# tk1363704/CAREL-VAE

Measured on AMD Instinct MI355X. Metric: clause-pairs/sec (training step), higher is better.
Workload: dtype bf16

## Files before the change

carel_vae_amd/csrc/rowvec_device.h:

```cpp
#pragma once
#include "carel_hip_internal.h"

namespace carel {

constexpr int TH = 768;
constexpr int TNV = TH / 256;

struct PtrSet4 { const float* w[4]; const float* b[4]; };

template <int ACT>
__global__ __launch_bounds__(256) void rowvec_linear_kernel(const float* __restrict__ in, long in_stride, const int* __restrict__ row_idx,
                                                            int B, int N, int seg, PtrSet4 ps, float* __restrict__ out, long out_stride) {
  const int lane = threadIdx.x & 63;
  const int n = blockIdx.x * 4 + (threadIdx.x >> 6);
  if (n >= N) return;
  const int bg = (B + gridDim.y - 1) / gridDim.y, b0 = blockIdx.y * bg, b1 = min(B, b0 + bg);
  const float* w = ps.w[n / seg] + (long)(n % seg) * TH;
  const float bias = ps.b[n / seg] ? ps.b[n / seg][n % seg] : 0.f;
  float4 wv[TNV];
#pragma unroll
  for (int i = 0; i < TNV; ++i) wv[i] = *(const float4*)(w + (i * 64 + lane) * 4);
  for (int b = b0; b < b1; b += 4) {
    float s[4];
#pragma unroll
    for (int u = 0; u < 4; ++u) {
      const int bb = min(b + u, b1 - 1);
      const float* x = row_idx ? in + (long)row_idx[bb] * TH : in + (long)bb * in_stride;
      float t = 0.f;
#pragma unroll
      for (int i = 0; i < TNV; ++i) {
        const float4 xv = *(const float4*)(x + (i * 64 + lane) * 4);
        t += (xv.x * wv[i].x + xv.y * wv[i].y) + (xv.z * wv[i].z + xv.w * wv[i].w);
      }
      s[u] = t;
    }
#pragma unroll
    for (int off = 32; off > 0; off >>= 1) {
#pragma unroll
      for (int u = 0; u < 4; ++u) s[u] += __shfl_xor(s[u], off, 64);
    }
#pragma unroll
    for (int u = 0; u < 4; ++u) {
      float v = s[u] + bias;
      if (ACT == 1) v = tanhf(v);
      if (lane == 0 && b + u < b1) out[(long)(b + u) * out_stride + n] = v;
    }
  }
}

struct OutSet4 { float* w[4]; float* b[4]; };
static __global__ __launch_bounds__(256) void rowvec_wgrad_kernel(const float* __restrict__ dY, long dy_stride, const float* __restrict__ X,
                                                           long x_stride, const int* __restrict__ row_idx, int B, int N, int seg, OutSet4 os) {
  const int lane = threadIdx.x & 63;
  const int n = blockIdx.x * 4 + (threadIdx.x >> 6);
  if (n >= N) return;
  float4 acc[TNV];
#pragma unroll
  for (int i = 0; i < TNV; ++i) acc[i] = float4{0.f, 0.f, 0.f, 0.f};
  float sb = 0.f;
  constexpr int U = 8;
  for (int b = 0; b < B; b += U) {
    float g[U]; float4 xv[U][TNV];
#pragma unroll
    for (int u = 0; u < U; ++u) {
      const int bb = min(b + u, B - 1);
      g[u] = (b + u < B) ? dY[(long)bb * dy_stride + n] : 0.f;
      const float* x = row_idx ? X + (long)row_idx[bb] * TH : X + (long)bb * x_stride;
#pragma unroll
      for (int i = 0; i < TNV; ++i) xv[u][i] = *(const float4*)(x + (i * 64 + lane) * 4);
    }
#pragma unroll
    for (int u = 0; u < U; ++u) {
      sb += g[u];
#pragma unroll
      for (int i = 0; i < TNV; ++i) {
        acc[i].x = fmaf(g[u], xv[u][i].x, acc[i].x); acc[i].y = fmaf(g[u], xv[u][i].y, acc[i].y);
        acc[i].z = fmaf(g[u], xv[u][i].z, acc[i].z); acc[i].w = fmaf(g[u], xv[u][i].w, acc[i].w);
      }
    }
  }
  float* w = os.w[n / seg] + (long)(n % seg) * TH;
#pragma unroll
  for (int i = 0; i < TNV; ++i) *(float4*)(w + (i * 64 + lane) * 4) = acc[i];
  if (lane == 0 && os.b[n / seg]) os.b[n / seg][n % seg] = sb;
}

constexpr int DG_CHUNK = 32;
template <int MODE>
__global__ __launch_bounds__(256) void rowvec_dgrad_kernel(const float* __restrict__ dY, long dy_stride, int B, int N, int seg,
                                                           PtrSet4 ps, const float* __restrict__ y, float* __restrict__ dpre,
                                                           float* __restrict__ part) {
  const int lane = threadIdx.x & 63;
  const int b = blockIdx.x * 4 + (threadIdx.x >> 6);
  if (b >= B) return;
  float4 acc[TNV];
#pragma unroll
  for (int i = 0; i < TNV; ++i) acc[i] = float4{0.f, 0.f, 0.f, 0.f};
  const int n0 = blockIdx.y * DG_CHUNK, n1 = min(N, n0 + DG_CHUNK);
  constexpr int U = 8;
  for (int nb = n0; nb < n1; nb += U) {
    float g[U]; float4 wv[U][TNV];
#pragma unroll
    for (int u = 0; u < U; ++u) {
      const int n = min(nb + u, n1 - 1);
      float gg = (nb + u < n1) ? dY[(long)b * dy_stride + n] : 0.f;
      if (MODE == 1) {
        const float yy = y[(long)b * N + n];
        gg *= (1.0f - yy * yy);
        if (lane == 0 && nb + u < n1) dpre[(long)b * N + n] = gg;
      }
      g[u] = gg;
      const float* w = ps.w[n / seg] + (long)(n % seg) * TH;
#pragma unroll
      for (int i = 0; i < TNV; ++i) wv[u][i] = *(const float4*)(w + (i * 64 + lane) * 4);
    }
#pragma unroll
    for (int u = 0; u < U; ++u) {
#pragma unroll
      for (int i = 0; i < TNV; ++i) {
        acc[i].x = fmaf(g[u], wv[u][i].x, acc[i].x); acc[i].y = fmaf(g[u], wv[u][i].y, acc[i].y);
        acc[i].z = fmaf(g[u], wv[u][i].z, acc[i].z); acc[i].w = fmaf(g[u], wv[u][i].w, acc[i].w);
      }
    }
  }
  float* o = part + ((long)blockIdx.y * B + b) * TH;
#pragma unroll
  for (int i = 0; i < TNV; ++i) *(float4*)(o + (i * 64 + lane) * 4) = acc[i];
}

static __global__ __launch_bounds__(256) void sum_parts_kernel(const float* __restrict__ part, float* __restrict__ out, long n, int nparts) {
  const long i = ((long)blockIdx.x * 256 + threadIdx.x) * 4;
  if (i >= n) return;
  float4 a = *(const float4*)(part + i);
  for (int p = 1; p < nparts; ++p) {
    const float4 b = *(const float4*)(part + (long)p * n + i);
    a.x += b.x; a.y += b.y; a.z += b.z; a.w += b.w;
  }
  *(float4*)(out + i) = a;
}

static __global__ void scale_inplace_kernel(float* __restrict__ x, long n, const float* __restrict__ scale) {
  const float s = scale[0];
  long i = (long)blockIdx.x * blockDim.x + threadIdx.x;
  const long stride = (long)gridDim.x * blockDim.x;
  for (; i < n; i += stride) x[i] *= s;
}
static __global__ __launch_bounds__(256) void scatter_cls_kernel(const float* __restrict__ dcls, int B, int S, const int* __restrict__ row_idx,
                                                          float* __restrict__ dx) {
  const int b = blockIdx.x;
  const long row = row_idx ? (long)row_idx[b] : (long)b * S;
  for (int k = threadIdx.x; k < TH; k += 256) dx[row * TH + k] = dcls[(long)b * TH + k];
}


}
```

carel_vae_amd/csrc/tail.hip:

```cpp
#include "carel_hip_internal.h"
#include "mmd_device.h"
#include "hsic_device.h"
#include "rowvec_device.h"

namespace carel {

struct TailCore {
  int B, D, EC;
  const float* lat;
  const float* eps_e; const float* eps_c;
  const float* emo_w; const float* emo_b;
  const float* cau_w; const float* cau_b;
  const float* pair_w; const float* pair_b;
  const long* emo_labels; const float* cau_labels; const float* pair_labels;
  float w_mmd, w_emo, w_cau, w_pair, kl_w, ls;
  int dis_mode;
  int emo_bce;
  Dropout d_emo, d_cau, d_pair;
  float alpha, mmd_eps;
  const float* label_sum_override; float n_override;
  int label_sum_ranks;
  const float* z_global; int n_global, row_offset; float mmd_grad_scale;
  int rank_stride;
  const float* mmd_part; int mmd_nblk; const float* dz_mmd;
// ... 350 lines not shown
  float ls;
  float* part;
  float* rowstat;
  float* dz_part;
  float* dw; float* db;
  float gscale;
};

template <int CD2>
__device__ __forceinline__ float dec_logit(const float* wr, const float* zrow, int D2rt, float bias) {
  const int D2 = CD2 ? CD2 : D2rt;
  float s = bias;
  if (CD2 && (CD2 & 3) == 0) {
#pragma unroll
    for (int k = 0; k < D2; k += 4) {
      const float4 zv = *(const float4*)(zrow + k);
      s = fmaf(wr[k], zv.x, s); s = fmaf(wr[k + 1], zv.y, s); s = fmaf(wr[k + 2], zv.z, s); s = fmaf(wr[k + 3], zv.w, s);
    }
  } else {
#pragma unroll
    for (int k = 0; k < D2; ++k) s = fmaf(wr[k], zrow[k], s);
  }
  return s;
}

template <int PASS, int CD2>
__global__ __launch_bounds__(DEC_J * DEC_MAXG) void decoder_kernel(DecArgs a) {
  const int D2 = CD2 ? CD2 : a.D2;
  const int ws = D2 + 1;
  extern __shared__ __attribute__((aligned(16))) char smem_raw[];
  float* zl = (float*)smem_raw;
  float* red = zl + a.B * D2;
  float* wl = red + 16;
  float* tile = wl + DEC_J * ws;
  float* tile2 = tile + a.B * DEC_J;
  const int t = threadIdx.x, nthr = blockDim.x, G = nthr / DEC_J;
  const int tj = t & (DEC_J - 1), g = t / DEC_J;
  const int j0 = blockIdx.x * DEC_J, j = j0 + tj;
  const bool live = j < a.V;
  const int Bg = (a.B + G - 1) / G, b0 = g * Bg, b1 = min(a.B, b0 + Bg);
  for (int e = t; e < a.B * D2; e += nthr) zl[e] = a.z[e];
  {
    const int nrow = min(DEC_J, a.V - j0);
    for (int e = t; e < nrow * D2; e += nthr) { const int r = e / D2, k = e - r * D2; wl[r * ws + k] = a.w[(long)j0 * D2 + e]; }
  }
  __syncthreads();
  float wr[CD2 ? CD2 : DEC_MAXD2];
  _Pragma("unroll") for (int k = 0; k < D2; ++k) wr[k] = live ? wl[tj * ws + k] : 0.f;
  const float bias = live ? a.b[j] : 0.f;
  const int lane = t & 63, wv = t >> 6, nwv = nthr >> 6;
  if (PASS == 1) {
    for (int b = b0; b < b1; ++b) tile[b * DEC_J + tj] = live ? dec_logit<CD2>(wr, zl + b * D2, D2, bias) : -INFINITY;
    __syncthreads();
    for (int b = wv; b < a.B; b += nwv) {
      const float x0 = tile[b * DEC_J + lane], x1 = tile[b * DEC_J + 64 + lane];
      const float m = wave_max(fmaxf(x0, x1));
      const float s2 = wave_sum(expf(x0 - m) + expf(x1 - m));
      if (lane == 0) { a.part[((long)blockIdx.x * a.B + b) * 2] = m; a.part[((long)blockIdx.x * a.B + b) * 2 + 1] = s2; }
    }
  } else if (PASS == 2) {
    for (int bb = b0; bb < b1; bb += 4) {
      float bw[4];
      _Pragma("unroll") for (int u = 0; u < 4; ++u) bw[u] = (live && bb + u < b1) ? a.bow[(long)(bb + u) * a.V + j] : 0.f;
      _Pragma("unroll") for (int u = 0; u < 4; ++u) {
        const int b = bb + u;
        if (b < b1) {
          float le = 0.f, dt = 0.f;
          if (live) {
            const float lp = dec_logit<CD2>(wr, zl + b * D2, D2, bias) - a.rowstat[b * 4] - a.rowstat[b * 4 + 1];
            const float p = expf(lp);
            const float tg = bw[u] * (1.f - a.ls) + a.ls / a.V;
            le = -(tg * fmaxf(lp, -100.f) + (1.f - tg) * fmaxf(log1pf(-p), -100.f));
            dt = p * ((p - tg) / fmaxf((1.f - p) * p, 1e-12f));
          }
          tile[b * DEC_J + tj] = le; tile2[b * DEC_J + tj] = dt;
        }
      }
    }
    __syncthreads();
    for (int b = wv; b < a.B; b += nwv) {
      const float le = wave_sum(tile[b * DEC_J + lane] + tile[b * DEC_J + 64 + lane]);
      const float dt = wave_sum(tile2[b * DEC_J + lane] + tile2[b * DEC_J + 64 + lane]);
      if (lane == 0) { a.part[((long)blockIdx.x * a.B + b) * 2] = le; a.part[((long)blockIdx.x * a.B + b) * 2 + 1] = dt; }
    }
  } else {
    float dwr[CD2 ? CD2 : DEC_MAXD2];
    _Pragma("unroll") for (int k = 0; k < D2; ++k) dwr[k] = 0.f;
    float dbj = 0.f;
    for (int bb = b0; bb < b1; bb += 4) {
      float bw[4];
      _Pragma("unroll") for (int u = 0; u < 4; ++u) bw[u] = (live && bb + u < b1) ? a.bow[(long)(bb + u) * a.V + j] : 0.f;
      _Pragma("unroll") for (int u = 0; u < 4; ++u) {
        const int b = bb + u;
        if (b < b1) {
          float gg = 0.f;
          if (live) {
            const float lp = dec_logit<CD2>(wr, zl + b * D2, D2, bias) - a.rowstat[b * 4] - a.rowstat[b * 4 + 1];
            const float p = expf(lp);
            const float tg = bw[u] * (1.f - a.ls) + a.ls / a.V;
            const float gp = (p - tg) / fmaxf((1.f - p) * p, 1e-12f);
            gg = p * (gp - a.rowstat[b * 4 + 2]) * a.gscale;
            _Pragma("unroll") for (int k = 0; k < D2; ++k) dwr[k] = fmaf(gg, zl[b * D2 + k], dwr[k]);
            dbj += gg;
          }
          tile[b * DEC_J + tj] = gg;
        }
      }
    }
    float* dwp = tile2;
    float* dbp = dwp + (G - 1) * DEC_J * ws;
    if (g > 0) {
      _Pragma("unroll") for (int k = 0; k < D2; ++k) dwp[((g - 1) * DEC_J + tj) * ws + k] = dwr[k];
      dbp[(g - 1) * DEC_J + tj] = dbj;
    }
    __syncthreads();
    if (g == 0 && live) {
      for (int q = 0; q < G - 1; ++q) {
        _Pragma("unroll") for (int k = 0; k < D2; ++k) dwr[k] += dwp[(q * DEC_J + tj) * ws + k];
        dbj += dbp[q * DEC_J + tj];
      }
      _Pragma("unroll") for (int k = 0; k < D2; ++k) a.dw[(long)j * D2 + k] = dwr[k];
      a.db[j] = dbj;
    }
    for (int e = t; e < a.B * D2; e += nthr) {
      const int b = e / D2, k = e - b * D2;
      const int nrow = min(DEC_J, a.V - j0);
      float s = 0.f;
      for (int jj = 0; jj < nrow; ++jj) s = fmaf(tile[b * DEC_J + jj], wl[jj * ws + k], s);
      a.dz_part[(long)blockIdx.x * a.B * D2 + e] = s;
    }
  }
}

__global__ __launch_bounds__(256) void decoder_combine_kernel(const float* __restrict__ part, int chunks, int B, int pass,
                                                              float* __restrict__ rowstat) {
  const int lane = threadIdx.x & 63;
  const int b = blockIdx.x * 4 + (threadIdx.x >> 6);
  if (b >= B) return;
  if (pass == 1) {
    float m = -INFINITY;
    for (int c = lane; c < chunks; c += 64) m = fmaxf(m, part[((long)c * B + b) * 2]);
    m = wave_max(m);
    float s = 0.f;
    for (int c = lane; c < chunks; c += 64) s += part[((long)c * B + b) * 2 + 1] * expf(part[((long)c * B + b) * 2] - m);
    s = wave_sum(s);
    if (lane == 0) { rowstat[b * 4] = m; rowstat[b * 4 + 1] = logf(s); }
  } else {
    float le = 0.f, dt = 0.f;
    for (int c = lane; c < chunks; c += 64) { le += part[((long)c * B + b) * 2]; dt += part[((long)c * B + b) * 2 + 1]; }
    le = wave_sum(le); dt = wave_sum(dt);
    if (lane == 0) { rowstat[b * 4 + 2] = dt; rowstat[b * 4 + 3] = le; }
  }
}
__global__ __launch_bounds__(256) void decoder_total_kernel(const float* __restrict__ rowstat, int B, float inv_bv, float* __restrict__ terms) {
  __shared__ float red[16];
  float tot = 0.f;
  for (int b = threadIdx.x; b < B; b += 256) tot += rowstat[b * 4 + 3];
  tot = block_sum(tot, red);
  if (threadIdx.x == 0) { terms[7] = tot * inv_bv; terms[8] = terms[0] + tot * inv_bv; }
}

__global__ __launch_bounds__(256) void reduce_parts16_kernel(const float* __restrict__ parts, float* __restrict__ out, int n, int nparts) {
  __shared__ float lds[256];
  const int cl = threadIdx.x & 15, rl = threadIdx.x >> 4;
  const int c = blockIdx.x * 16 + cl;
  float s = 0.f;
  if (c < n) for (int p = rl; p < nparts; p += 16) s += parts[(long)p * n + c];
  lds[threadIdx.x] = s;
  __syncthreads();
  if (rl == 0 && c < n) {
    float t = 0.f;
#pragma unroll
    for (int r = 0; r < 16; ++r) t += lds[r * 16 + cl];
    out[c] = t;
  }
}

__global__ __launch_bounds__(256) void tail_dlat_kernel(const float* __restrict__ dz_core, const float* __restrict__ dz_part, int chunks,
                                                        const float* __restrict__ dlat_direct, const float* __restrict__ lat,
                                                        const float* __restrict__ eps_e, const float* __restrict__ eps_c, int B, int D,
                                                        float gout, float* __restrict__ dlat) {
  const int e = blockIdx.x * 256 + threadIdx.x;
  if (e >= B * 2 * D) return;
  const int b = e / (2 * D), k = e - b * 2 * D;
  float g = dz_core[e];
  for (int c = 0; c < chunks; ++c) g += dz_part[(long)c * B * 2 * D + e];
  const int side = k >= D, kk = k - side * D;
  const float* row = lat + (long)b * 4 * D;
  const float ep = side ? eps_c[kk] : eps_e[kk];
  const float lv = row[(2 * side + 1) * D + kk];
  dlat[(long)b * 4 * D + 2 * side * D + kk] = (dlat_direct[(long)b * 4 * D + 2 * side * D + kk] + g) * gout;
  dlat[(long)b * 4 * D + (2 * side + 1) * D + kk] = (dlat_direct[(long)b * 4 * D + (2 * side + 1) * D + kk] + g * ep * expf(lv)) * gout;
}

__global__ __launch_bounds__(256) void sample_z_kernel(const float* __restrict__ lat, const float* __restrict__ eps_e,
                                                       const float* __restrict__ eps_c, int B, int D, float* __restrict__ z) {
  const int e = blockIdx.x * 256 + threadIdx.x;
  if (e >= B * 2 * D) return;
  const int b = e / (2 * D), k = e - b * 2 * D;
  const float* row = lat + (long)b * 4 * D;
  z[e] = (k < D) ? row[k] + eps_e[k] * expf(row[D + k]) : row[2 * D + (k - D)] + eps_c[k - D] * expf(row[3 * D + (k - D)]);
}

__global__ __launch_bounds__(256) void pair_prob_kernel(const float* __restrict__ lat, const float* __restrict__ eps_e,
                                                        const float* __restrict__ eps_c, const float* __restrict__ w,
                                                        const float* __restrict__ bias, int B, int D, float* __restrict__ prob) {
  const int b = blockIdx.x * 256 + threadIdx.x;
  if (b >= B) return;
  const float* row = lat + (long)b * 4 * D;
  float s = bias[0];
  for (int k = 0; k < D; ++k) {
    s = fmaf(w[k], row[k] + eps_e[k] * expf(row[D + k]), s);
    s = fmaf(w[D + k], row[2 * D + k] + eps_c[k] * expf(row[3 * D + k]), s);
  }
  prob[b] = 1.0f / (1.0f + expf(-s));
}

}

using namespace carel;

static size_t align_up(size_t x) { return (x + 63) & ~(size_t)63; }
constexpr int MMD_MAX_BLOCKS = 1024;

struct TailWork {
  float* dz_core; float* dlat_direct; float* dlat; float* dpooled; float* dpre; float* part; float* rowstat; float* dz_part;
  float* dcls; float* dgpart; float* pair_dead; float* mmd_part; float* dz_mmd;
  size_t total;
};
static TailWork carve(float* base, int B, int D, int V) {
  TailWork w; size_t o = 0;
  const int chunks = (V + DEC_J - 1) / DEC_J;
  auto take = [&](size_t n) { float* p = base ? base + o : nullptr; o += align_up(n); return p; };
  w.dz_core = take((size_t)B * 2 * D); w.dlat_direct = take((size_t)B * 4 * D); w.dlat = take((size_t)B * 4 * D);
  w.dpooled = take((size_t)B * TH); w.dpre = take((size_t)B * TH); w.part = take((size_t)chunks * B * 2);
  w.rowstat = take((size_t)B * 4); w.dz_part = take((size_t)chunks * B * 2 * D); w.dcls = take((size_t)B * TH);
  w.dgpart = take((size_t)((TH + DG_CHUNK - 1) / DG_CHUNK) * B * TH);
  w.pair_dead = take(16);
  w.mmd_part = take(4 * MMD_MAX_BLOCKS); w.dz_mmd = take((size_t)B * 2 * D);
  w.total = o;
  return w;
}

extern "C" int64_t carel_tail_workspace_floats(int32_t batch, int32_t ec_dim, int32_t bow_dim) {
  return (int64_t)carve(nullptr, batch, ec_dim, bow_dim).total;
}

static int tail_check(const carel_tail_args* a, const char* who) {
  if (!a) return set_error(CAREL_ERR_ARG, "%s: null args", who);
  if (a->hidden != TH) return set_error(CAREL_ERR_SHAPE, "%s: hidden must be %d", who, TH);
  if (a->batch < 1 || a->seq_len < 1) return set_error(CAREL_ERR_SHAPE, "%s: bad batch/seq_len", who);
  if (a->ec_dim < 1 || a->ec_dim > 32 || a->e_classes < 1 || a->e_classes > 8)
    return set_error(CAREL_ERR_SHAPE, "%s: ec_dim must be <= 32 and e_num_class <= 8", who);
  if (!a->x_last_f32 || !a->pooler_w || !a->pooler_b || !a->pooled || !a->lat)
    return set_error(CAREL_ERR_ARG, "%s: null tensor", who);
  for (int i = 0; i < 4; ++i) if (!a->head_w[i] || !a->head_b[i]) return set_error(CAREL_ERR_ARG, "%s: null latent head", who);
  return CAREL_OK;
}

extern "C" int carel_tail_latents(const carel_tail_args* a, void* stream_) {
  hipStream_t stream = (hipStream_t)stream_;
  int rc = tail_check(a, "carel_tail_latents");
  if (rc) return rc;
  auto sample_groups = [&](int ncols) { int g = (4096 + ncols - 1) / ncols;       const int mx = (a->batch + 3) / 4; g = g > mx ? mx : g; return g < 1 ? 1 : g; };
  const int N = 4 * a->ec_dim;
  if (a->head_in_f32) {
    const int N2 = 2 * a->ec_dim;
    for (int side = 0; side < 2; ++side) {
      PtrSet4 hp; for (int i = 0; i < 4; ++i) { hp.w[i] = nullptr; hp.b[i] = nullptr; }
      for (int i = 0; i < 2; ++i) { hp.w[i] = (const float*)a->head_w[2 * side + i]; hp.b[i] = (const float*)a->head_b[2 * side + i]; }
      hipLaunchKernelGGL(rowvec_linear_kernel<0>, dim3((N2 + 3) / 4, sample_groups(N2)), dim3(256), 0, stream,
                         (const float*)a->head_in_f32 + (long)side * a->batch * TH, (long)TH, (const int*)nullptr, a->batch, N2, a->ec_dim, hp,
                         (float*)a->lat + side * N2, (long)N);
    }
  } else {
    PtrSet4 pp; for (int i = 0; i < 4; ++i) { pp.w[i] = nullptr; pp.b[i] = nullptr; }
    pp.w[0] = (const float*)a->pooler_w; pp.b[0] = (const float*)a->pooler_b;
    hipLaunchKernelGGL(rowvec_linear_kernel<1>, dim3(TH / 4, sample_groups(TH)), dim3(256), 0, stream, (const float*)a->x_last_f32,
                       (long)a->seq_len * TH, (const int*)a->cls_rows, a->batch, TH, TH, pp, (float*)a->pooled, (long)TH);
    PtrSet4 hp; for (int i = 0; i < 4; ++i) { hp.w[i] = (const float*)a->head_w[i]; hp.b[i] = (const float*)a->head_b[i]; }
    hipLaunchKernelGGL(rowvec_linear_kernel<0>, dim3((N + 3) / 4, sample_groups(N)), dim3(256), 0, stream, (const float*)a->pooled, (long)TH,
                       (const int*)nullptr, a->batch, N, a->ec_dim, hp, (float*)a->lat, (long)N);
  }
  if (a->eps_e && a->eps_c && a->z)
    hipLaunchKernelGGL(sample_z_kernel, dim3((a->batch * 2 * a->ec_dim + 255) / 256), dim3(256), 0, stream, (const float*)a->lat,
                       (const float*)a->eps_e, (const float*)a->eps_c, a->batch, a->ec_dim, (float*)a->z);
  return check_launch("tail latents");
}

extern "C" int carel_pair_probs(const void* lat, const void* eps_e, const void* eps_c, const void* pair_w, const void* pair_b,
                                int32_t batch, int32_t ec_dim, void* prob, void* stream_) {
  hipStream_t stream = (hipStream_t)stream_;
  if (!lat || !eps_e || !eps_c || !pair_w || !pair_b || !prob || batch < 1) return set_error(CAREL_ERR_ARG, "carel_pair_probs: bad arguments");
  hipLaunchKernelGGL(pair_prob_kernel, dim3((batch + 255) / 256), dim3(256), 0, stream, (const float*)lat, (const float*)eps_e,
                     (const float*)eps_c, (const float*)pair_w, (const float*)pair_b, batch, ec_dim, (float*)prob);
  return check_launch("pair_prob_kernel");
}

extern "C" int carel_tail_losses(const carel_tail_args* a, void* stream_) {
  hipStream_t stream = (hipStream_t)stream_;
  int rc = tail_check(a, "carel_tail_losses");
  if (rc) return rc;
  const int B = a->batch, D = a->ec_dim, V = a->bow_dim;
  if (V < 1) return set_error(CAREL_ERR_SHAPE, "carel_tail_losses: bow_dim must be positive");
  if (2 * D > DEC_MAXD2) return set_error(CAREL_ERR_SHAPE, "carel_tail_losses: 2*ec_dim must be <= %d", DEC_MAXD2);
  if (B > 1024) return set_error(CAREL_ERR_SHAPE, "carel_tail_losses: batch must be <= 1024 per rank");
  if (B < 2 && !a->z_global) return set_error(CAREL_ERR_SHAPE, "carel_tail_losses: batch must be >= 2 (MMD divides by n(n-1))");
  if (!a->emo_w || !a->emo_b || !a->cau_w || !a->cau_b || !a->pair_w || !a->pair_b || !a->dec_w || !a->dec_b ||
      !a->emo_labels || !a->cau_labels || !a->pair_labels || !a->bow || !a->eps_e || !a->eps_c || !a->z || !a->terms ||
      !a->work || !a->d_emo_w || !a->d_emo_b || !a->d_cau_w || !a->d_cau_b || !a->d_pair_w || !a->d_pair_b || !a->d_dec_w ||
      !a->d_dec_b)
    return set_error(CAREL_ERR_ARG, "carel_tail_losses: null tensor");
  TailWork w = carve((float*)a->work, B, D, V);
  TailCore c;
  c.B = B; c.D = D; c.EC = a->e_classes; c.lat = (const float*)a->lat; c.eps_e = (const float*)a->eps_e; c.eps_c = (const float*)a->eps_c;
  c.emo_w = (const float*)a->emo_w; c.emo_b = (const float*)a->emo_b; c.cau_w = (const float*)a->cau_w; c.cau_b = (const float*)a->cau_b;
  c.pair_w = (const float*)a->pair_w; c.pair_b = (const float*)a->pair_b;
  c.emo_labels = (const long*)a->emo_labels; c.cau_labels = (const float*)a->cau_labels; c.pair_labels = (const float*)a->pair_labels;
  c.w_mmd = a->w_mmd; c.w_emo = a->w_emo; c.w_cau = a->w_cau; c.w_pair = a->w_pair; c.kl_w = a->kl_weight; c.ls = a->label_smoothing;
  c.dis_mode = a->dis_mode; c.emo_bce = a->emo_bce;
  if (c.dis_mode < 0 || c.dis_mode > 2) return set_error(CAREL_ERR_ARG, "carel_tail_losses: dis_mode must be 0 (MMD), 1 (HSIC) or 2 (none)");
  if (c.emo_bce && a->e_classes != 1) return set_error(CAREL_ERR_ARG, "carel_tail_losses: the BCE emotion head has exactly one logit");
  if (c.dis_mode == 1 && a->z_global) return set_error(CAREL_ERR_ARG, "carel_tail_losses: HSIC has no global-batch mode");
  c.d_emo = make_dropout(a->drop_seed, 100u, a->drop_p, a->drop_row_offset * (uint32_t)D);
  c.d_cau = make_dropout(a->drop_seed, 101u, a->drop_p, a->drop_row_offset * (uint32_t)D);
  c.d_pair = make_dropout(a->drop_seed, 102u, a->drop_p, a->drop_row_offset * (uint32_t)(2 * D));
  c.alpha = a->mmd_alpha; c.mmd_eps = a->mmd_eps;
  c.label_sum_override = (const float*)a->global_label_sum; c.n_override = (float)a->global_n;
  c.label_sum_ranks = a->global_label_ranks > 1 ? a->global_label_ranks : 1;
  if (c.label_sum_ranks > 1 && a->global_rank_stride <= 0)
    return set_error(CAREL_ERR_ARG, "carel_tail_losses: global_label_ranks > 1 needs global_rank_stride");
  c.z_global = (const float*)a->z_global; c.n_global = a->global_n; c.row_offset = a->global_row_offset;
  c.rank_stride = a->global_rank_stride > 0 ? a->global_rank_stride : B * 2 * D;
  if (c.z_global && a->global_rank_stride > 0 && (a->global_rank_stride < B * 2 * D || c.n_global % B))
    return set_error(CAREL_ERR_ARG, "carel_tail_losses: global_rank_stride needs global_n to be a multiple of batch and stride >= batch*2*ec_dim");
  c.mmd_grad_scale = a->mmd_grad_scale > 0.f ? a->mmd_grad_scale : 1.f;
  if (c.z_global && (c.n_global < 2 || c.row_offset < 0 || c.row_offset + B > c.n_global))
    return set_error(CAREL_ERR_ARG, "carel_tail_losses: inconsistent global batch description");
  c.z = (float*)a->z; c.terms = (float*)a->terms; c.dz = w.dz_core; c.dlat_direct = w.dlat_direct;
  c.d_emo_w = (float*)a->d_emo_w; c.d_emo_b = (float*)a->d_emo_b; c.d_cau_w = (float*)a->d_cau_w; c.d_cau_b = (float*)a->d_cau_b;
  c.d_pair_w = (float*)a->d_pair_w; c.d_pair_b = (float*)a->d_pair_b; c.pair_dead = w.pair_dead;
  const int nm = (c.z_global && c.dis_mode != 0) ? c.n_global : B;
  const int n_hw = a->e_classes * D + a->e_classes + D + 1 + 2 * D + 1;
  const size_t lds = sizeof(float) * (64 + 64 + (size_t)2 * B * 2 * D + (size_t)B * 8 + (size_t)B * 2 + (size_t)B * 4 * D + (size_t)B * 16 +
                                      ((n_hw + 3) & ~3) + ((2 * nm + 3) & ~3) + (size_t)2 * nm * (D | 1) + 2 * (size_t)B);
  if (lds > 160 * 1024) return set_error(CAREL_ERR_SHAPE, "carel_tail_losses: batch too large for the single-workgroup tail (%zu B LDS)", lds);
  if (lds > 64 * 1024) {
    hipError_t e = hipFuncSetAttribute((const void*)tail_core_kernel, hipFuncAttributeMaxDynamicSharedMemorySize, (int)lds);
    if (e != hipSuccess) return set_error(CAREL_ERR_HIP, "carel_tail_losses: hipFuncSetAttribute: %s", hipGetErrorString(e));
  }
  c.mmd_part = nullptr; c.mmd_nblk = 0; c.dz_mmd = nullptr;
  if (c.z_global && c.dis_mode == 0 && (2 * c.n_global + 31) / 32 > MMD_MAX_BLOCKS)
    return set_error(CAREL_ERR_SHAPE, "carel_tail_losses: global batch too large for the MMD partial buffer");
  hipStream_t core_stream = stream;
  TailEvents* tev = nullptr;
  auto join_on_error = [&](int code) -> int {
    if (tev && core_stream != stream) {
      (void)hipEventRecord(tev->join, core_stream);
      (void)hipStreamWaitEvent(stream, tev->join, 0);
    }
    return code;
  };
  if (g_tail_overlap && !a->serial && !g_tail_prof) {
    hipStream_t side = (hipStream_t)carel_side_stream(0);
    tev = side ? tail_events() : nullptr;
    if (tev) {
      hipLaunchKernelGGL(sample_z_kernel, dim3((B * 2 * D + 255) / 256), dim3(256), 0, stream, c.lat, c.eps_e, c.eps_c, B, D, c.z);
      if (hipEventRecord(tev->fork, stream) != hipSuccess || hipStreamWaitEvent(side, tev->fork, 0) != hipSuccess)
        return set_error(CAREL_ERR_HIP, "carel_tail_losses: event fork failed");
      core_stream = side;
      c.z = nullptr;
    }
  }
  if (c.z_global && c.dis_mode == 0) {
    MmdGlobalArgs g;
    g.zg = c.z_global; g.n = c.n_global; g.B = B; g.D = D; g.rank_stride = c.rank_stride; g.row_offset = c.row_offset;
    g.alpha = c.alpha; g.eps = c.mmd_eps; g.gscale = -c.w_mmd * c.mmd_grad_scale; g.part = w.mmd_part; g.dz = w.dz_mmd;
    const int nblk = (2 * c.n_global + 31) / 32;
    if (D == 24) hipLaunchKernelGGL(mmd_global_kernel<24>, dim3(nblk), dim3(256), 0, core_stream, g);
    else hipLaunchKernelGGL(mmd_global_kernel<32>, dim3(nblk), dim3(256), 0, core_stream, g);
    if ((rc = check_launch("mmd_global_kernel"))) return join_on_error(rc);
    c.mmd_part = w.mmd_part; c.mmd_nblk = nblk; c.dz_mmd = w.dz_mmd;
  }
  c.prof = g_tail_prof;
  hipLaunchKernelGGL(tail_core_kernel, dim3(1), dim3(1024), lds, core_stream, c);
  if ((rc = check_launch("tail_core_kernel"))) return join_on_error(rc);
  if (tev && hipEventRecord(tev->join, core_stream) != hipSuccess) return set_error(CAREL_ERR_HIP, "carel_tail_losses: event record failed");

  DecArgs d;
  d.B = B; d.D2 = 2 * D; d.V = V; d.z = (const float*)a->z; d.w = (const float*)a->dec_w; d.b = (const float*)a->dec_b;
  d.bow = (const float*)a->bow; d.ls = a->label_smoothing; d.part = w.part; d.rowstat = w.rowstat; d.dz_part = w.dz_part;
  d.dw = (float*)a->d_dec_w; d.db = (float*)a->d_dec_b; d.gscale = 1.0f / ((float)B * (float)V);
  const int chunks = (V + DEC_J - 1) / DEC_J;
  const size_t lds0 = sizeof(float) * ((size_t)B * 2 * D + 16 + (size_t)DEC_J * (2 * D + 1) + (size_t)B * DEC_J);
  int G = DEC_MAXG;
  auto lds3_of = [&](int g) { return lds0 + sizeof(float) * (size_t)(g - 1) * DEC_J * (2 * D + 2); };
  while (G > 1 && (lds3_of(G) > 160 * 1024 || (B + G - 1) / G < 4)) G >>= 1;
  const size_t lds1 = lds0, lds2 = lds0 + sizeof(float) * (size_t)B * DEC_J, lds3 = lds3_of(G);
  const size_t ldsmax = lds2 > lds3 ? lds2 : lds3;
  if (ldsmax > 160 * 1024) return set_error(CAREL_ERR_SHAPE, "carel_tail_losses: batch too large for the decoder kernel");
  if (ldsmax > 64 * 1024) {
    hipError_t e = hipSuccess;
    const void* fns[6] = {(const void*)decoder_kernel<1, 48>, (const void*)decoder_kernel<2, 48>, (const void*)decoder_kernel<3, 48>,
                          (const void*)decoder_kernel<1, 0>, (const void*)decoder_kernel<2, 0>, (const void*)decoder_kernel<3, 0>};
    for (int i = 0; i < 6 && e == hipSuccess; ++i) e = hipFuncSetAttribute(fns[i], hipFuncAttributeMaxDynamicSharedMemorySize, (int)ldsmax);
    if (e != hipSuccess) return set_error(CAREL_ERR_HIP, "carel_tail_losses: hipFuncSetAttribute: %s", hipGetErrorString(e));
  }
#define DEC_LAUNCH(PASS, LDS)                                                                              \
  do {                                                                                                  \
    if (2 * D == 48) hipLaunchKernelGGL((decoder_kernel<PASS, 48>), dim3(chunks), dim3(DEC_J * G), LDS, stream, d); \
    else hipLaunchKernelGGL((decoder_kernel<PASS, 0>), dim3(chunks), dim3(DEC_J * G), LDS, stream, d);      \
  } while (0)
  DEC_LAUNCH(1, lds1);
  hipLaunchKernelGGL(decoder_combine_kernel, dim3((B + 3) / 4), dim3(256), 0, stream, (const float*)w.part, chunks, B, 1, w.rowstat);
  DEC_LAUNCH(2, lds2);
  hipLaunchKernelGGL(decoder_combine_kernel, dim3((B + 3) / 4), dim3(256), 0, stream, (const float*)w.part, chunks, B, 2, w.rowstat);
  DEC_LAUNCH(3, lds3);
#undef DEC_LAUNCH
  if ((rc = check_launch("decoder kernels"))) return rc;
  hipLaunchKernelGGL(reduce_parts16_kernel, dim3((B * 2 * D + 15) / 16), dim3(256), 0, stream, (const float*)w.dz_part, w.dz_part, B * 2 * D, chunks);
  if (tev && hipStreamWaitEvent(stream, tev->join, 0) != hipSuccess) return set_error(CAREL_ERR_HIP, "carel_tail_losses: event join failed");
  hipLaunchKernelGGL(decoder_total_kernel, dim3(1), dim3(256), 0, stream, (const float*)w.rowstat, B, d.gscale, (float*)a->terms);
  hipLaunchKernelGGL(tail_dlat_kernel, dim3((B * 2 * D + 255) / 256), dim3(256), 0, stream, (const float*)w.dz_core, (const float*)w.dz_part,
                     1, (const float*)w.dlat_direct, (const float*)a->lat, (const float*)a->eps_e, (const float*)a->eps_c, B, D, 1.0f, w.dlat);
  return check_launch("tail_dlat_kernel");
}

extern "C" int carel_scale_f32(void* x, int64_t n, const void* scale_dev, void* stream_) {
  hipStream_t stream = (hipStream_t)stream_;
  if (!x || !scale_dev || n <= 0) return set_error(CAREL_ERR_ARG, "carel_scale_f32: bad arguments");
  long blocks = (n + 255) / 256; if (blocks > 2048) blocks = 2048;
  hipLaunchKernelGGL(scale_inplace_kernel, dim3((unsigned)blocks), dim3(256), 0, stream, (float*)x, (long)n, (const float*)scale_dev);
  return check_launch("scale_inplace_kernel");
}

__global__ void bow_scatter_kernel(const int* __restrict__ rows, const int* __restrict__ cols, const float* __restrict__ vals, int nnz,
                                   float* __restrict__ out, int B, int V) {
  const int i = blockIdx.x * blockDim.x + threadIdx.x;
  if (i >= nnz) return;
  const int r = rows[i], c = cols[i];
  if (r >= 0 && r < B && c >= 0 && c < V) out[(long)r * V + c] = vals[i];
}
extern "C" int carel_bow_expand(const void* trip, int32_t nnz, void* out, int32_t B, int32_t V, void* stream_) {
  hipStream_t stream = (hipStream_t)stream_;
  if (!out || B < 1 || V < 1 || nnz < 0 || (nnz > 0 && !trip)) return set_error(CAREL_ERR_ARG, "carel_bow_expand: bad arguments");
  hipError_t e = hipMemsetAsync(out, 0, (size_t)B * V * 4, stream);
  if (e != hipSuccess) return set_error(CAREL_ERR_HIP, "carel_bow_expand: memset: %s", hipGetErrorString(e));
  if (nnz == 0) return CAREL_OK;
  const int* rows = (const int*)trip;
  hipLaunchKernelGGL(bow_scatter_kernel, dim3((nnz + 255) / 256), dim3(256), 0, stream, rows, rows + nnz, (const float*)(rows + 2 * (long)nnz), nnz,
                     (float*)out, B, V);
  return check_launch("bow_scatter_kernel");
}

extern "C" int64_t carel_tail_pair_dead_offset(int32_t batch, int32_t ec_dim, int32_t bow_dim) {
  TailWork w = carve((float*)nullptr + 1, batch, ec_dim, bow_dim);
  return (int64_t)(w.pair_dead - ((float*)nullptr + 1));
}

extern "C" int carel_tail_profile(void* dev_i64_x16) { g_tail_prof = (long long*)dev_i64_x16; return CAREL_OK; }

extern "C" int carel_tail_backward(const carel_tail_args* a, const void* grad_out_dev, void* stream_) {
  return carel_tail_backward_dz(a, grad_out_dev, nullptr, stream_);
}

__global__ __launch_bounds__(256) void tail_add_dz_kernel(const float* __restrict__ dz, const float* __restrict__ lat,
                                                          const float* __restrict__ eps_e, const float* __restrict__ eps_c, int B, int D,
                                                          float* __restrict__ dlat) {
  const int e = blockIdx.x * 256 + threadIdx.x;
  if (e >= B * 2 * D) return;
  const int b = e / (2 * D), k = e - b * 2 * D, side = k >= D, kk = k - side * D;
  const float g = dz[e];
  const float ep = side ? eps_c[kk] : eps_e[kk];
  const float lv = lat[(long)b * 4 * D + (2 * side + 1) * D + kk];
  dlat[(long)b * 4 * D + 2 * side * D + kk] += g;
  dlat[(long)b * 4 * D + (2 * side + 1) * D + kk] += g * ep * expf(lv);
}

extern "C" int carel_tail_backward_dz(const carel_tail_args* a, const void* grad_out_dev, const void* dz_extra, void* stream_) {
  hipStream_t stream = (hipStream_t)stream_;
  int rc = tail_check(a, "carel_tail_backward");
  if (rc) return rc;
  if (!a->work || !a->dx_last_f32 || !a->d_pooler_w || !a->d_pooler_b) return set_error(CAREL_ERR_ARG, "carel_tail_backward: null tensor");
  const int B = a->batch, D = a->ec_dim, N = 4 * D;
  TailWork w = carve((float*)a->work, B, D, a->bow_dim);
  if (grad_out_dev) {
    hipLaunchKernelGGL(scale_inplace_kernel, dim3((B * N + 255) / 256), dim3(256), 0, stream, w.dlat, (long)B * N, (const float*)grad_out_dev);
  }
  if (dz_extra) {
    if (!a->lat || !a->eps_e || !a->eps_c) return set_error(CAREL_ERR_ARG, "carel_tail_backward_dz: lat / eps needed");
    hipLaunchKernelGGL(tail_add_dz_kernel, dim3((B * 2 * D + 255) / 256), dim3(256), 0, stream, (const float*)dz_extra, (const float*)a->lat,
                       (const float*)a->eps_e, (const float*)a->eps_c, B, D, w.dlat);
  }
  const int hc = (N + DG_CHUNK - 1) / DG_CHUNK, pc = (TH + DG_CHUNK - 1) / DG_CHUNK;
  const long bt = (long)B * TH;
  if (a->head_in_f32) {
    if (!a->d_head_in_f32) return set_error(CAREL_ERR_ARG, "carel_tail_backward: head_in_f32 needs d_head_in_f32");
    const int N2 = 2 * D, hc2 = (N2 + DG_CHUNK - 1) / DG_CHUNK;
    for (int side = 0; side < 2; ++side) {
      PtrSet4 hp; OutSet4 ho;
      for (int i = 0; i < 4; ++i) { hp.w[i] = nullptr; hp.b[i] = nullptr; ho.w[i] = nullptr; ho.b[i] = nullptr; }
      for (int i = 0; i < 2; ++i) { hp.w[i] = (const float*)a->head_w[2 * side + i]; ho.w[i] = (float*)a->d_head_w[2 * side + i]; ho.b[i] = (float*)a->d_head_b[2 * side + i]; }
      const float* hin = (const float*)a->head_in_f32 + side * bt;
      if (ho.w[0] && ho.w[1])
        hipLaunchKernelGGL(rowvec_wgrad_kernel, dim3((N2 + 3) / 4), dim3(256), 0, stream, (const float*)w.dlat + side * N2, (long)N, hin,
                           (long)TH, (const int*)nullptr, B, N2, D, ho);
      hipLaunchKernelGGL(rowvec_dgrad_kernel<0>, dim3((B + 3) / 4, hc2), dim3(256), 0, stream, (const float*)w.dlat + side * N2, (long)N, B, N2, D, hp,
                         (const float*)nullptr, (float*)nullptr, w.dgpart);
      hipLaunchKernelGGL(sum_parts_kernel, dim3((unsigned)((bt / 4 + 255) / 256)), dim3(256), 0, stream, (const float*)w.dgpart,
                         (float*)a->d_head_in_f32 + side * bt, bt, hc2);
    }
    (void)hipMemsetAsync(a->d_pooler_w, 0, (size_t)TH * TH * sizeof(float), stream);
    (void)hipMemsetAsync(a->d_pooler_b, 0, (size_t)TH * sizeof(float), stream);
    return check_launch("tail backward (adapter heads)");
  }
  PtrSet4 hp; OutSet4 ho;
  for (int i = 0; i < 4; ++i) { hp.w[i] = (const float*)a->head_w[i]; hp.b[i] = nullptr; ho.w[i] = (float*)a->d_head_w[i]; ho.b[i] = (float*)a->d_head_b[i]; }
  if (ho.w[0] && ho.w[1] && ho.w[2] && ho.w[3])
    hipLaunchKernelGGL(rowvec_wgrad_kernel, dim3((N + 3) / 4), dim3(256), 0, stream, (const float*)w.dlat, (long)N, (const float*)a->pooled,
                       (long)TH, (const int*)nullptr, B, N, D, ho);
  hipLaunchKernelGGL(rowvec_dgrad_kernel<0>, dim3((B + 3) / 4, hc), dim3(256), 0, stream, (const float*)w.dlat, (long)N, B, N, D, hp,
                     (const float*)nullptr, (float*)nullptr, w.dgpart);
  hipLaunchKernelGGL(sum_parts_kernel, dim3((unsigned)((bt / 4 + 255) / 256)), dim3(256), 0, stream, (const float*)w.dgpart, w.dpooled, bt, hc);
  PtrSet4 pp; OutSet4 po;
  for (int i = 0; i < 4; ++i) { pp.w[i] = nullptr; pp.b[i] = nullptr; po.w[i] = nullptr; po.b[i] = nullptr; }
  pp.w[0] = (const float*)a->pooler_w; po.w[0] = (float*)a->d_pooler_w; po.b[0] = (float*)a->d_pooler_b;
  hipLaunchKernelGGL(rowvec_dgrad_kernel<1>, dim3((B + 3) / 4, pc), dim3(256), 0, stream, (const float*)w.dpooled, (long)TH, B, TH, TH, pp,
                     (const float*)a->pooled, w.dpre, w.dgpart);
  hipLaunchKernelGGL(sum_parts_kernel, dim3((unsigned)((bt / 4 + 255) / 256)), dim3(256), 0, stream, (const float*)w.dgpart, w.dcls, bt, pc);
  hipLaunchKernelGGL(rowvec_wgrad_kernel, dim3(TH / 4), dim3(256), 0, stream, (const float*)w.dpre, (long)TH, (const float*)a->x_last_f32,
                     (long)a->seq_len * TH, (const int*)a->cls_rows, B, TH, TH, po);
  const size_t dx_rows = a->n_rows > 0 ? (size_t)a->n_rows : (size_t)B * a->seq_len;
  (void)hipMemsetAsync(a->dx_last_f32, 0, dx_rows * TH * sizeof(float), stream);
  hipLaunchKernelGGL(scatter_cls_kernel, dim3(B), dim3(256), 0, stream, (const float*)w.dcls, B, a->seq_len, (const int*)a->cls_rows,
                     (float*)a->dx_last_f32);
  return check_launch("tail backward");
}
```

Baseline: 8302.

## Fuse tail backward reductions into consumers and merge wgrad and scatter launches

Drops the separate sum_parts passes: dgrad kernels now read partial sums directly through a DySrc that adds the parts and applies the grad scale on load. The two weight-grad launches become one combined grid, and memset plus CLS scatter become a single expand kernel that writes zeros or summed grads. In the forward tail, the parts reduction, decoder total and dlat kernels merge into one finish kernel, and the side-stream sample_z launch is removed. This trades fewer launches and less intermediate traffic for repeated part summation inside inner loops and a per-row ballot search over cls_rows.

```diff
diff --git a/carel_vae_amd/csrc/rowvec_device.h b/carel_vae_amd/csrc/rowvec_device.h
--- a/carel_vae_amd/csrc/rowvec_device.h
+++ b/carel_vae_amd/csrc/rowvec_device.h
@@ -48,11 +48,23 @@
   }
 }
 
+struct DySrc { const float* p; long stride; int nparts; long pstride; const float* scale; };
+static inline DySrc dy_src(const float* p, long stride, int nparts = 1, long pstride = 0, const float* scale = nullptr) {
+  DySrc d; d.p = p; d.stride = stride; d.nparts = nparts; d.pstride = pstride; d.scale = scale; return d;
+}
+__device__ __forceinline__ float dy_at(const DySrc& d, int b, int n) {
+  const long i = (long)b * d.stride + n;
+  float v = d.p[i];
+  for (int q = 1; q < d.nparts; ++q) v += d.p[(long)q * d.pstride + i];
+  if (d.scale) v *= d.scale[0];
+  return v;
+}
+
 struct OutSet4 { float* w[4]; float* b[4]; };
-static __global__ __launch_bounds__(256) void rowvec_wgrad_kernel(const float* __restrict__ dY, long dy_stride, const float* __restrict__ X,
-                                                           long x_stride, const int* __restrict__ row_idx, int B, int N, int seg, OutSet4 os) {
-  const int lane = threadIdx.x & 63;
-  const int n = blockIdx.x * 4 + (threadIdx.x >> 6);
+__device__ __forceinline__ void rowvec_wgrad_body(DySrc dY, const float* __restrict__ X, long x_stride, const int* __restrict__ row_idx,
+                                                  int B, int N, int seg, OutSet4 os, int blk) {
+  const int lane = threadIdx.x & 63;
+  const int n = blk * 4 + (threadIdx.x >> 6);
   if (n >= N) return;
   float4 acc[TNV];
 #pragma unroll
@@ -64,7 +76,7 @@
 #pragma unroll
     for (int u = 0; u < U; ++u) {
       const int bb = min(b + u, B - 1);
-      g[u] = (b + u < B) ? dY[(long)bb * dy_stride + n] : 0.f;
+      g[u] = (b + u < B) ? dy_at(dY, bb, n) : 0.f;
       const float* x = row_idx ? X + (long)row_idx[bb] * TH : X + (long)bb * x_stride;
 #pragma unroll
       for (int i = 0; i < TNV; ++i) xv[u][i] = *(const float4*)(x + (i * 64 + lane) * 4);
@@ -79,17 +91,27 @@
       }
     }
   }
-  float* w = os.w[n / seg] + (long)(n % seg) * TH;
+  const int h = n / seg;
+  float* w = (h == 0 ? os.w[0] : h == 1 ? os.w[1] : h == 2 ? os.w[2] : os.w[3]) + (long)(n % seg) * TH;
+  float* ob = h == 0 ? os.b[0] : h == 1 ? os.b[1] : h == 2 ? os.b[2] : os.b[3];
 #pragma unroll
   for (int i = 0; i < TNV; ++i) *(float4*)(w + (i * 64 + lane) * 4) = acc[i];
-  if (lane == 0 && os.b[n / seg]) os.b[n / seg][n % seg] = sb;
+  if (lane == 0 && ob) ob[n % seg] = sb;
+}
+static __global__ __launch_bounds__(256) void rowvec_wgrad_kernel(const float* __restrict__ dY, long dy_stride, const float* __restrict__ X,
+                                                           long x_stride, const int* __restrict__ row_idx, int B, int N, int seg, OutSet4 os) {
+  rowvec_wgrad_body(DySrc{dY, dy_stride, 1, 0, nullptr}, X, x_stride, row_idx, B, N, seg, os, blockIdx.x);
+}
+struct WgradProb { DySrc dy; const float* X; long x_stride; const int* row_idx; int N, seg; OutSet4 os; };
+static __global__ __launch_bounds__(256) void rowvec_wgrad2_kernel(WgradProb p0, WgradProb p1, int nblk0, int B) {
+  if ((int)blockIdx.x < nblk0) rowvec_wgrad_body(p0.dy, p0.X, p0.x_stride, p0.row_idx, B, p0.N, p0.seg, p0.os, blockIdx.x);
+  else rowvec_wgrad_body(p1.dy, p1.X, p1.x_stride, p1.row_idx, B, p1.N, p1.seg, p1.os, blockIdx.x - nblk0);
 }
 
 constexpr int DG_CHUNK = 32;
 template <int MODE>
-__global__ __launch_bounds__(256) void rowvec_dgrad_kernel(const float* __restrict__ dY, long dy_stride, int B, int N, int seg,
-                                                           PtrSet4 ps, const float* __restrict__ y, float* __restrict__ dpre,
-                                                           float* __restrict__ part) {
+__device__ __forceinline__ void rowvec_dgrad_body(const DySrc& dY, int B, int N, int seg, const PtrSet4& ps, const float* __restrict__ y,
+                                                  float* __restrict__ dpre, float* __restrict__ part) {
   const int lane = threadIdx.x & 63;
   const int b = blockIdx.x * 4 + (threadIdx.x >> 6);
   if (b >= B) return;
@@ -103,7 +125,7 @@
 #pragma unroll
     for (int u = 0; u < U; ++u) {
       const int n = min(nb + u, n1 - 1);
-      float gg = (nb + u < n1) ? dY[(long)b * dy_stride + n] : 0.f;
+      float gg = (nb + u < n1) ? dy_at(dY, b, n) : 0.f;
       if (MODE == 1) {
         const float yy = y[(long)b * N + n];
         gg *= (1.0f - yy * yy);
@@ -126,6 +148,17 @@
   float* o = part + ((long)blockIdx.y * B + b) * TH;
 #pragma unroll
   for (int i = 0; i < TNV; ++i) *(float4*)(o + (i * 64 + lane) * 4) = acc[i];
+}
+template <int MODE>
+__global__ __launch_bounds__(256) void rowvec_dgrad_kernel(const float* __restrict__ dY, long dy_stride, int B, int N, int seg,
+                                                           PtrSet4 ps, const float* __restrict__ y, float* __restrict__ dpre,
+                                                           float* __restrict__ part) {
+  rowvec_dgrad_body<MODE>(DySrc{dY, dy_stride, 1, 0, nullptr}, B, N, seg, ps, y, dpre, part);
+}
+template <int MODE>
+__global__ __launch_bounds__(256) void rowvec_dgrad_src_kernel(DySrc dY, int B, int N, int seg, PtrSet4 ps, const float* __restrict__ y,
+                                                               float* __restrict__ dpre, float* __restrict__ part) {
+  rowvec_dgrad_body<MODE>(dY, B, N, seg, ps, y, dpre, part);
 }
 
 static __global__ __launch_bounds__(256) void sum_parts_kernel(const float* __restrict__ part, float* __restrict__ out, long n, int nparts) {
@@ -152,5 +185,34 @@
   for (int k = threadIdx.x; k < TH; k += 256) dx[row * TH + k] = dcls[(long)b * TH + k];
 }
 
-
-}
+static __global__ __launch_bounds__(256) void cls_expand_kernel(const float* __restrict__ part, int nparts, int B, int S,
+                                                               const int* __restrict__ row_idx, long rows, float* __restrict__ dx) {
+  const long r = (long)blockIdx.x * 4 + (threadIdx.x >> 6);
+  const int lane = threadIdx.x & 63;
+  if (r >= rows) return;
+  int b = -1;
+  if (row_idx) {
+    for (int j0 = 0; j0 < B && b < 0; j0 += 64) {
+      const unsigned long long hit = __ballot(j0 + lane < B && row_idx[j0 + lane] == r);
+      if (hit) b = j0 + __ffsll((long long)hit) - 1;
+    }
+  } else if (r % S == 0 && r / S < B) {
+    b = (int)(r / S);
+  }
+  const long n = (long)B * TH;
+#pragma unroll
+  for (int i = 0; i < TNV; ++i) {
+    const int k = (i * 64 + lane) * 4;
+    float4 v = float4{0.f, 0.f, 0.f, 0.f};
+    if (b >= 0) {
+      v = *(const float4*)(part + (long)b * TH + k);
+      for (int p = 1; p < nparts; ++p) {
+        const float4 q = *(const float4*)(part + (long)p * n + (long)b * TH + k);
+        v.x += q.x; v.y += q.y; v.z += q.z; v.w += q.w;
+      }
+    }
+    *(float4*)(dx + r * TH + k) = v;
+  }
+}
+
+}
diff --git a/carel_vae_amd/csrc/tail.hip b/carel_vae_amd/csrc/tail.hip
--- a/carel_vae_amd/csrc/tail.hip
+++ b/carel_vae_amd/csrc/tail.hip
@@ -526,45 +526,40 @@
     if (lane == 0) { rowstat[b * 4 + 2] = dt; rowstat[b * 4 + 3] = le; }
   }
 }
-__global__ __launch_bounds__(256) void decoder_total_kernel(const float* __restrict__ rowstat, int B, float inv_bv, float* __restrict__ terms) {
+__global__ __launch_bounds__(256) void tail_finish_kernel(const float* __restrict__ dz_core, const float* __restrict__ dz_part, int chunks,
+                                                          const float* __restrict__ dlat_direct, const float* __restrict__ lat,
+                                                          const float* __restrict__ eps_e, const float* __restrict__ eps_c, int B, int D,
+                                                          float* __restrict__ dlat, const float* __restrict__ rowstat, float inv_bv,
+                                                          float* __restrict__ terms) {
+  __shared__ float lds[256];
   __shared__ float red[16];
-  float tot = 0.f;
-  for (int b = threadIdx.x; b < B; b += 256) tot += rowstat[b * 4 + 3];
-  tot = block_sum(tot, red);
-  if (threadIdx.x == 0) { terms[7] = tot * inv_bv; terms[8] = terms[0] + tot * inv_bv; }
-}
-
-__global__ __launch_bounds__(256) void reduce_parts16_kernel(const float* __restrict__ parts, float* __restrict__ out, int n, int nparts) {
-  __shared__ float lds[256];
+  const int n = B * 2 * D;
   const int cl = threadIdx.x & 15, rl = threadIdx.x >> 4;
-  const int c = blockIdx.x * 16 + cl;
+  const int e = blockIdx.x * 16 + cl;
   float s = 0.f;
-  if (c < n) for (int p = rl; p < nparts; p += 16) s += parts[(long)p * n + c];
+  if (e < n) for (int p = rl; p < chunks; p += 16) s += dz_part[(long)p * n + e];
   lds[threadIdx.x] = s;
   __syncthreads();
-  if (rl == 0 && c < n) {
+  if (rl == 0 && e < n) {
     float t = 0.f;
 #pragma unroll
     for (int r = 0; r < 16; ++r) t += lds[r * 16 + cl];
-    out[c] = t;
-  }
-}
-
-__global__ __launch_bounds__(256) void tail_dlat_kernel(const float* __restrict__ dz_core, const float* __restrict__ dz_part, int chunks,
-                                                        const float* __restrict__ dlat_direct, const float* __restrict__ lat,
-                                                        const float* __restrict__ eps_e, const float* __restrict__ eps_c, int B, int D,
-                                                        float gout, float* __restrict__ dlat) {
-  const int e = blockIdx.x * 256 + threadIdx.x;
-  if (e >= B * 2 * D) return;
-  const int b = e / (2 * D), k = e - b * 2 * D;
-  float g = dz_core[e];
-  for (int c = 0; c < chunks; ++c) g += dz_part[(long)c * B * 2 * D + e];
-  const int side = k >= D, kk = k - side * D;
-  const float* row = lat + (long)b * 4 * D;
-  const float ep = side ? eps_c[kk] : eps_e[kk];
-  const float lv = row[(2 * side + 1) * D + kk];
-  dlat[(long)b * 4 * D + 2 * side * D + kk] = (dlat_direct[(long)b * 4 * D + 2 * side * D + kk] + g) * gout;
-  dlat[(long)b * 4 * D + (2 * side + 1) * D + kk] = (dlat_direct[(long)b * 4 * D + (2 * side + 1) * D + kk] + g * ep * expf(lv)) * gout;
+    float g = dz_core[e];
+    g += t;
+    const int b = e / (2 * D), k = e - b * 2 * D;
+    const int side = k >= D, kk = k - side * D;
+    const float* row = lat + (long)b * 4 * D;
+    const float ep = side ? eps_c[kk] : eps_e[kk];
+    const float lv = row[(2 * side + 1) * D + kk];
+    dlat[(long)b * 4 * D + 2 * side * D + kk] = dlat_direct[(long)b * 4 * D + 2 * side * D + kk] + g;
+    dlat[(long)b * 4 * D + (2 * side + 1) * D + kk] = dlat_direct[(long)b * 4 * D + (2 * side + 1) * D + kk] + g * ep * expf(lv);
+  }
+  if (blockIdx.x == 0) {
+    float tot = 0.f;
+    for (int b = threadIdx.x; b < B; b += 256) tot += rowstat[b * 4 + 3];
+    tot = block_sum(tot, red);
+    if (threadIdx.x == 0) { terms[7] = tot * inv_bv; terms[8] = terms[0] + tot * inv_bv; }
+  }
 }
 
 __global__ __launch_bounds__(256) void sample_z_kernel(const float* __restrict__ lat, const float* __restrict__ eps_e,
@@ -598,8 +593,8 @@
 constexpr int MMD_MAX_BLOCKS = 1024;
 
 struct TailWork {
-  float* dz_core; float* dlat_direct; float* dlat; float* dpooled; float* dpre; float* part; float* rowstat; float* dz_part;
-  float* dcls; float* dgpart; float* pair_dead; float* mmd_part; float* dz_mmd;
+  float* dz_core; float* dlat_direct; float* dlat; float* dpre; float* part; float* rowstat; float* dz_part;
+  float* dgpart; float* pair_dead; float* mmd_part; float* dz_mmd; float* dhpart;
   size_t total;
 };
 static TailWork carve(float* base, int B, int D, int V) {
@@ -607,11 +602,12 @@
   const int chunks = (V + DEC_J - 1) / DEC_J;
   auto take = [&](size_t n) { float* p = base ? base + o : nullptr; o += align_up(n); return p; };
   w.dz_core = take((size_t)B * 2 * D); w.dlat_direct = take((size_t)B * 4 * D); w.dlat = take((size_t)B * 4 * D);
-  w.dpooled = take((size_t)B * TH); w.dpre = take((size_t)B * TH); w.part = take((size_t)chunks * B * 2);
-  w.rowstat = take((size_t)B * 4); w.dz_part = take((size_t)chunks * B * 2 * D); w.dcls = take((size_t)B * TH);
+  w.dpre = take((size_t)B * TH); w.part = take((size_t)chunks * B * 2);
+  w.rowstat = take((size_t)B * 4); w.dz_part = take((size_t)chunks * B * 2 * D);
   w.dgpart = take((size_t)((TH + DG_CHUNK - 1) / DG_CHUNK) * B * TH);
   w.pair_dead = take(16);
   w.mmd_part = take(4 * MMD_MAX_BLOCKS); w.dz_mmd = take((size_t)B * 2 * D);
+  w.dhpart = take((size_t)((4 * D + DG_CHUNK - 1) / DG_CHUNK) * B * TH);
   w.total = o;
   return w;
 }
@@ -739,7 +735,6 @@
     hipStream_t side = (hipStream_t)carel_side_stream(0);
     tev = side ? tail_events() : nullptr;
     if (tev) {
-      hipLaunchKernelGGL(sample_z_kernel, dim3((B * 2 * D + 255) / 256), dim3(256), 0, stream, c.lat, c.eps_e, c.eps_c, B, D, c.z);
       if (hipEventRecord(tev->fork, stream) != hipSuccess || hipStreamWaitEvent(side, tev->fork, 0) != hipSuccess)
         return set_error(CAREL_ERR_HIP, "carel_tail_losses: event fork failed");
       core_stream = side;
@@ -792,12 +787,11 @@
   DEC_LAUNCH(3, lds3);
 #undef DEC_LAUNCH
   if ((rc = check_launch("decoder kernels"))) return rc;
-  hipLaunchKernelGGL(reduce_parts16_kernel, dim3((B * 2 * D + 15) / 16), dim3(256), 0, stream, (const float*)w.dz_part, w.dz_part, B * 2 * D, chunks);
   if (tev && hipStreamWaitEvent(stream, tev->join, 0) != hipSuccess) return set_error(CAREL_ERR_HIP, "carel_tail_losses: event join failed");
-  hipLaunchKernelGGL(decoder_total_kernel, dim3(1), dim3(256), 0, stream, (const float*)w.rowstat, B, d.gscale, (float*)a->terms);
-  hipLaunchKernelGGL(tail_dlat_kernel, dim3((B * 2 * D + 255) / 256), dim3(256), 0, stream, (const float*)w.dz_core, (const float*)w.dz_part,
-                     1, (const float*)w.dlat_direct, (const float*)a->lat, (const float*)a->eps_e, (const float*)a->eps_c, B, D, 1.0f, w.dlat);
-  return check_launch("tail_dlat_kernel");
+  hipLaunchKernelGGL(tail_finish_kernel, dim3((B * 2 * D + 15) / 16), dim3(256), 0, stream, (const float*)w.dz_core, (const float*)w.dz_part,
+                     chunks, (const float*)w.dlat_direct, (const float*)a->lat, (const float*)a->eps_e, (const float*)a->eps_c, B, D, w.dlat,
+                     (const float*)w.rowstat, d.gscale, (float*)a->terms);
+  return check_launch("tail_finish_kernel");
 }
 
 extern "C" int carel_scale_f32(void* x, int64_t n, const void* scale_dev, void* stream_) {
@@ -858,8 +852,11 @@
   if (!a->work || !a->dx_last_f32 || !a->d_pooler_w || !a->d_pooler_b) return set_error(CAREL_ERR_ARG, "carel_tail_backward: null tensor");
   const int B = a->batch, D = a->ec_dim, N = 4 * D;
   TailWork w = carve((float*)a->work, B, D, a->bow_dim);
-  if (grad_out_dev) {
+  const float* dlat_scale = nullptr;
+  if (grad_out_dev && (dz_extra || a->head_in_f32)) {
     hipLaunchKernelGGL(scale_inplace_kernel, dim3((B * N + 255) / 256), dim3(256), 0, stream, w.dlat, (long)B * N, (const float*)grad_out_dev);
+  } else {
+    dlat_scale = (const float*)grad_out_dev;
   }
   if (dz_extra) {
     if (!a->lat || !a->eps_e || !a->eps_c) return set_error(CAREL_ERR_ARG, "carel_tail_backward_dz: lat / eps needed");
@@ -890,23 +887,22 @@
   }
   PtrSet4 hp; OutSet4 ho;
   for (int i = 0; i < 4; ++i) { hp.w[i] = (const float*)a->head_w[i]; hp.b[i] = nullptr; ho.w[i] = (float*)a->d_head_w[i]; ho.b[i] = (float*)a->d_head_b[i]; }
-  if (ho.w[0] && ho.w[1] && ho.w[2] && ho.w[3])
-    hipLaunchKernelGGL(rowvec_wgrad_kernel, dim3((N + 3) / 4), dim3(256), 0, stream, (const float*)w.dlat, (long)N, (const float*)a->pooled,
-                       (long)TH, (const int*)nullptr, B, N, D, ho);
-  hipLaunchKernelGGL(rowvec_dgrad_kernel<0>, dim3((B + 3) / 4, hc), dim3(256), 0, stream, (const float*)w.dlat, (long)N, B, N, D, hp,
-                     (const float*)nullptr, (float*)nullptr, w.dgpart);
-  hipLaunchKernelGGL(sum_parts_kernel, dim3((unsigned)((bt / 4 + 255) / 256)), dim3(256), 0, stream, (const float*)w.dgpart, w.dpooled, bt, hc);
+  const DySrc dlat = dy_src(w.dlat, N, 1, 0, dlat_scale);
+  hipLaunchKernelGGL(rowvec_dgrad_src_kernel<0>, dim3((B + 3) / 4, hc), dim3(256), 0, stream, dlat, B, N, D, hp, (const float*)nullptr,
+                     (float*)nullptr, w.dhpart);
   PtrSet4 pp; OutSet4 po;
   for (int i = 0; i < 4; ++i) { pp.w[i] = nullptr; pp.b[i] = nullptr; po.w[i] = nullptr; po.b[i] = nullptr; }
   pp.w[0] = (const float*)a->pooler_w; po.w[0] = (float*)a->d_pooler_w; po.b[0] = (float*)a->d_pooler_b;
-  hipLaunchKernelGGL(rowvec_dgrad_kernel<1>, dim3((B + 3) / 4, pc), dim3(256), 0, stream, (const float*)w.dpooled, (long)TH, B, TH, TH, pp,
+  hipLaunchKernelGGL(rowvec_dgrad_src_kernel<1>, dim3((B + 3) / 4, pc), dim3(256), 0, stream, dy_src(w.dhpart, TH, hc, bt), B, TH, TH, pp,
                      (const float*)a->pooled, w.dpre, w.dgpart);
-  hipLaunchKernelGGL(sum_parts_kernel, dim3((unsigned)((bt / 4 + 255) / 256)), dim3(256), 0, stream, (const float*)w.dgpart, w.dcls, bt, pc);
-  hipLaunchKernelGGL(rowvec_wgrad_kernel, dim3(TH / 4), dim3(256), 0, stream, (const float*)w.dpre, (long)TH, (const float*)a->x_last_f32,
-                     (long)a->seq_len * TH, (const int*)a->cls_rows, B, TH, TH, po);
-  const size_t dx_rows = a->n_rows > 0 ? (size_t)a->n_rows : (size_t)B * a->seq_len;
-  (void)hipMemsetAsync(a->dx_last_f32, 0, dx_rows * TH * sizeof(float), stream);
-  hipLaunchKernelGGL(scatter_cls_kernel, dim3(B), dim3(256), 0, stream, (const float*)w.dcls, B, a->seq_len, (const int*)a->cls_rows,
-                     (float*)a->dx_last_f32);
+  WgradProb wh, wp;
+  wh.dy = dlat; wh.X = (const float*)a->pooled; wh.x_stride = TH; wh.row_idx = nullptr; wh.N = N; wh.seg = D; wh.os = ho;
+  wp.dy = dy_src(w.dpre, TH); wp.X = (const float*)a->x_last_f32; wp.x_stride = (long)a->seq_len * TH; wp.row_idx = (const int*)a->cls_rows;
+  wp.N = TH; wp.seg = TH; wp.os = po;
+  const int nbh = (ho.w[0] && ho.w[1] && ho.w[2] && ho.w[3]) ? (N + 3) / 4 : 0;
+  hipLaunchKernelGGL(rowvec_wgrad2_kernel, dim3(nbh + TH / 4), dim3(256), 0, stream, wh, wp, nbh, B);
+  const long dx_rows = a->n_rows > 0 ? (long)a->n_rows : (long)B * a->seq_len;
+  hipLaunchKernelGGL(cls_expand_kernel, dim3((unsigned)((dx_rows + 3) / 4)), dim3(256), 0, stream, (const float*)w.dgpart, pc, B, a->seq_len,
+                     (const int*)a->cls_rows, dx_rows, (float*)a->dx_last_f32);
   return check_launch("tail backward");
 }
```

Result: no change. 8293 (median of 4 runs) (-0.1%).
